# gcorso/disco-diffdock

Hardware: AMD Instinct MI355X
Metric: complexes/sec, 20-step 40-sample inference (higher is better)
Workload: dtype f32

## Files before the change

disco_diffdock_amd/csrc/conv_launch.hip:

```cpp
#include "k_conv_common.h"
#include "k_node.h"
#include "model.h"

namespace ddk {

__global__ void conv_setup_kernel(int32_t* tile_info, int g0, int g1, int g2, int g3, int g4) {
  if (threadIdx.x == 0 && blockIdx.x == 0) {
    const int go[5] = {g0, g1, g2, g3, g4};
    int ts = 0;
    tile_info[0] = 0;
    for (int g = 0; g < 4; ++g) {
      ts += (go[g + 1] - go[g] + 31) / 32;
      tile_info[g + 1] = ts;
    }
    for (int g = 0; g < 5; ++g) tile_info[5 + g] = go[g];
    tile_info[10] = 0;
  }
}

__global__ void conv_one_group_kernel(int32_t* gt, int n_groups, int k, int E) {
  const int g = threadIdx.x;
  if (g < n_groups) { gt[g] = 0; gt[n_groups + g] = g == k ? E : 0; }
}

// ... 164 lines not shown
}

static ConvXArgs conv_args(const ConvLayerDev& L, const ConvLaunch& a, bool f16, bool trace) {
  ConvXArgs X = {};
  ConvKArgs& k = X.k;
  k.x = a.x; k.src = a.src; k.dst = a.dst; k.edge_attr = a.edge_attr; k.sh = a.sh; k.sum = a.sum;
  k.counter = a.counter;
  k.b1p = L.b1p[0]; k.n_tiles = L.n_tiles;
  k.n_cols = L.n_cols;
  for (int c = 0; c <= L.n_cols; ++c) k.col_start[c] = L.col_start[c];
  k.sum_g2 = a.sum_g2; k.g2_node_off = a.g2_node_off;
  k.n_groups = a.n_groups; k.n_active = a.n_active; k.n_slots = a.n_slots; k.slots = a.slots; k.wmap = a.wmap;
  if (a.gbeg) { k.gbeg = a.gbeg; k.gend = a.gend; }
  else { k.gbeg = a.tile_info + 5; k.gend = a.tile_info + 6; }
  k.pre = a.pre; k.part = a.part; k.det_rng = a.det_rng; k.det_nr = a.det_nr;
  if (f16) {
    k.w1x = L.w1x; k.w1sx = L.w1sx; k.w2x = L.w2x;
    for (int g = 0; g < CONV_MAX_GROUPS; ++g) { k.w1s[g] = L.w1s[g]; k.w1u[g] = 1.0f / L.w1s[g]; k.w2s[g] = L.w2s[g]; k.w2u[g] = 1.0f / L.w2s[g]; }
  } else {
    k.w1p = L.w1p[0]; k.w2r = L.w2r[0];
    for (int g = 0; g < CONV_MAX_GROUPS; ++g) { k.w1s[g] = 1.0f; k.w1u[g] = 1.0f; k.w2s[g] = 1.0f; k.w2u[g] = 1.0f; }
  }
  X.trace = trace ? a.trace : nullptr; X.trace_coarse = a.trace_coarse;
  return X;
}

hipError_t conv_prepare_device() {
  for (int family = CONV_F32; family <= CONV_X2; ++family) {
    const ConvTable t = conv_table(family);
    for (int i = 0; i < t.n; ++i) {
// ... 30 lines not shown
```

disco_diffdock_amd/csrc/ddk_internal.h:

```cpp
#pragma once
#include <hip/hip_runtime.h>
#include <stdint.h>

#include <map>
#include <string>
#include <vector>

#include "../../include/ddk.h"
#include "../../include/ddk_debug.h"

namespace ddk {

constexpr int NS = 24;
constexpr int NV = 6;
constexpr int XW = 2 * NS + 6 * NV;
constexpr int NE = 3 * NS;
constexpr int OFF_P = NS;
constexpr int OFF_Q = NS + 3 * NV;
constexpr int OFF_C = NS + 6 * NV;

constexpr int F_A = 0;
constexpr int F_C = NS;
constexpr int F_T1O = 2 * NS;
constexpr int F_T1E = F_T1O + 6 * NV;
// ... 189 lines not shown
  const int32_t* src;
  const int32_t* dst;
  const float* edge_attr;
  const float* sh;
  float* sum;
  const int32_t* tile_info;
  int32_t* counter;
  float* part = nullptr;
  int64_t edge_bound = 0;
  const int32_t* det_rng = nullptr;
  int det_nr = 0;
  const float* pre = nullptr;
  int gather;
  float* sum_g2 = nullptr;
  int g2_node_off = 0;
  int mode = 0;
  int n_groups = 4, n_active = 4, n_slots = 1;
  uint32_t slots = 0;
  uint64_t wmap = 0x876543210ull;
  const int32_t* gbeg = nullptr;
  const int32_t* gend = nullptr;
  uint32_t* trace = nullptr;
  int trace_coarse = 0;
};
hipError_t launch_conv_fused(const ConvLayerDev& L, const ConvLaunch& a, int n_cu, hipStream_t s);
hipError_t launch_split3_probe(const float* x, int64_t n, int group, float* hi, float* mid, float* lo, float* scale, hipStream_t s);
int build_conv_layer(ddk_ctx* ctx, int mode, int l, ConvLayerDev& L);
int build_head_layer(ddk_ctx* ctx, int mode, ConvLayerDev& L);
hipError_t conv_prepare_device();
hipError_t graph_prepare_device(int* max_rec);
// ... 141 lines not shown
```

disco_diffdock_amd/csrc/k_conv.hip:

```cpp
#include <stdlib.h>

#include "k_conv_common.h"

namespace ddk {

__device__ __forceinline__ void load_frags(float4 (&a)[9], f32x16& B, const float* w, const float* b) {
#pragma unroll
  for (int s4 = 0; s4 < 9; ++s4) a[s4] = ld4(w + s4 * 256);
#pragma unroll
  for (int j = 0; j < 4; ++j) {
    const float4 v = ld4(b + 4 * j);
    B[4 * j + 0] = v.x; B[4 * j + 1] = v.y; B[4 * j + 2] = v.z; B[4 * j + 3] = v.w;
  }
}

__device__ __forceinline__ f32x16 burst(const float4 (&a)[9], const float (&h)[36], const f32x16& C) {
  f32x16 D = MFMA(a[0].x, h[0], C);
  D = MFMA(a[0].y, h[1], D);
  D = MFMA(a[0].z, h[2], D);
  D = MFMA(a[0].w, h[3], D);
#pragma unroll
  for (int s4 = 1; s4 < 9; ++s4) {
    D = MFMA(a[s4].x, h[4 * s4 + 0], D);
    D = MFMA(a[s4].y, h[4 * s4 + 1], D);
// ... 14 lines not shown
}

template <bool GATHER, int MODE, bool SPLIT, bool DET>
__global__ __launch_bounds__(64 * ConvTraits<MODE>::WAVES) void conv_fused_kernel(ConvKArgs A) {
  static_assert(!SPLIT || (GATHER && MODE == 0), "the GEMM1 split exists for the score model's gather path");
  static_assert(!DET || MODE == 0, "the deterministic scatter exists for the score model");
  constexpr int WAVES = ConvTraits<MODE>::WAVES, FS = ConvTraits<MODE>::FS, BLOCK_EDGES = 32 * WAVES;
  extern __shared__ __attribute__((aligned(16))) float lds[];
  const int tid = threadIdx.x, lane = tid & 63, wave = tid >> 6;
  float* F = lds + wave * (32 * FS);
  float* ring = lds + WAVES * (32 * FS);
  int* blk_slot = reinterpret_cast<int*>(ring + 2 * W2_TILE_FLOATS);
  const int el = lane & 31;
  const int hh = lane >> 5;
  const bool g2_shared = A.sum_g2 != nullptr;
  int gb_v = 0, ge_v = 0;
  if (lane < A.n_active) {
    gb_v = A.gbeg[lane];
    ge_v = A.gend[lane];
  }
  const int nb_v = (ge_v - gb_v + BLOCK_EDGES - 1) / BLOCK_EDGES;
  int pend_v = nb_v;
#pragma unroll
  for (int d = 1; d < 16; d *= 2) {
    const int t = __shfl_up(pend_v, d, 64);
    if (lane >= d) pend_v += t;
  }
  const int pbeg_v = pend_v - nb_v;
  int bs4 = __builtin_amdgcn_readlane(pend_v, 15);
  if constexpr (DET) {
// ... 32 lines not shown
    }
    int g = __popcll(__ballot(lane < 16 && blk >= pend_v));
    int gbeg = __builtin_amdgcn_readlane(gb_v, g), gend = __builtin_amdgcn_readlane(ge_v, g);
    int bstart = __builtin_amdgcn_readlane(pbeg_v, g);
    if constexpr (DET) {
      if (A.det_nr > 0) {
        const DetRange R_ = det_find(A.det_rng, A.det_nr, blk);
        g = R_.g; gbeg = R_.beg; gend = R_.end; bstart = R_.bstart;
      }
    }
    const int e0 = gbeg + BLOCK_EDGES * (blk - bstart) + 32 * wave;
    const int nvalid = min(32, gend - e0);
    const bool valid = el < nvalid;
    const int e = nvalid > 0 ? e0 + min(el, nvalid - 1) : gend - 1;
    const int sn = A.src[e], dn = A.dst[e];

    const int gw = (int)((A.wmap >> (4 * g)) & 15);
    const float* wrec = A.w2r + (size_t)gw * n_tiles * W2_TILE_FLOATS;
    {
      const float* wr0 = wrec + (size_t)t_begin * W2_TILE_FLOATS;
      const float* wr1 = wrec + (size_t)min(t_begin + 1, t_end - 1) * W2_TILE_FLOATS;
      const float4 r0 = ld4(wr0 + 4 * tid), r1 = ld4(wr1 + 4 * tid);
      *reinterpret_cast<float4*>(ring + 4 * tid) = r0;
      *reinterpret_cast<float4*>(ring + W2_TILE_FLOATS + 4 * tid) = r1;
      if (second) {
        const int q = 4 * (tid + 64 * WAVES);
        const float4 r2 = ld4(wr0 + q), r3 = ld4(wr1 + q);
        *reinterpret_cast<float4*>(ring + q) = r2;
        *reinterpret_cast<float4*>(ring + W2_TILE_FLOATS + q) = r3;
      }
    }

    const SegCtl seg = make_segctl(sn, el, nvalid, valid);

    float h[36];
    if constexpr (SPLIT) {
      float bin[12];
      {
        const float* pe = A.edge_attr + (size_t)e * NS + 12 * hh;
#pragma unroll
        for (int j = 0; j < 3; ++j) {
          const float4 a = ld4(pe + 4 * j);
          bin[4 * j + 0] = a.x; bin[4 * j + 1] = a.y; bin[4 * j + 2] = a.z; bin[4 * j + 3] = a.w;
        }
      }
      const float* ps = A.pre + ((size_t)sn * 4 + (gw & 1)) * NE + 36 * hh;
      const float* pd = A.pre + ((size_t)dn * 4 + 2 + (gw >> 1)) * NE + 36 * hh;
      const float* w1 = A.w1p + (size_t)gw * (3 * 9 * 64 * 4);
#pragma unroll
      for (int T = 0; T < 3; ++T) {
        f32x16 acc;
#pragma unroll
        for (int j = 0; j < 4; ++j) {
          if (T < 2 || j == 0) {
// ... 13 lines not shown
          acc = MFMA(a.w, bin[4 * s4 + 3], acc);
        }
        if (T < 2) {
#pragma unroll
          for (int r = 0; r < 16; ++r) h[16 * T + r] = fmaxf(acc[r], 0.0f);
        } else {
#pragma unroll
          for (int r = 0; r < 4; ++r) h[32 + r] = fmaxf(acc[r], 0.0f);
        }
      }
    } else {
    float bin[36];
    {
      const float *pe, *pxs, *pxd;
      if (GATHER) {
        pe = A.edge_attr + (size_t)e * NS + 12 * hh;
        pxs = A.x + (size_t)sn * XW + 12 * hh;
        pxd = A.x + (size_t)dn * XW + 12 * hh;
      } else {
        pe = A.edge_attr + (size_t)e * NE + 12 * hh;
        pxs = pe + NS;
        pxd = pe + 2 * NS;
      }
#pragma unroll
      for (int j = 0; j < 3; ++j) {
        const float4 a = ld4(pe + 4 * j), b = ld4(pxs + 4 * j), c = ld4(pxd + 4 * j);
        bin[4 * j + 0] = a.x; bin[4 * j + 1] = a.y; bin[4 * j + 2] = a.z; bin[4 * j + 3] = a.w;
        bin[12 + 4 * j + 0] = b.x; bin[12 + 4 * j + 1] = b.y; bin[12 + 4 * j + 2] = b.z; bin[12 + 4 * j + 3] = b.w;
        bin[24 + 4 * j + 0] = c.x; bin[24 + 4 * j + 1] = c.y; bin[24 + 4 * j + 2] = c.z; bin[24 + 4 * j + 3] = c.w;
      }
    }
// ... 17 lines not shown
          acc = MFMA(a.y, bin[4 * s4 + 1], acc);
          acc = MFMA(a.z, bin[4 * s4 + 2], acc);
          acc = MFMA(a.w, bin[4 * s4 + 3], acc);
        }
        if (T < 2) {
#pragma unroll
          for (int r = 0; r < 16; ++r) h[16 * T + r] = fmaxf(acc[r], 0.0f);
        } else {
#pragma unroll
          for (int r = 0; r < 4; ++r) h[32 + r] = fmaxf(acc[r], 0.0f);
        }
      }
    }
    }

    const float4 shv = ld4(A.sh + (size_t)e * 4);
    const float s0 = shv.x, vx = shv.y, vy = shv.z, vz = shv.w;
    {
      const float* xr = A.x + (size_t)dn * XW;
      const int o_main_src = hh ? OFF_C : 0, o_main_dst = hh ? F_C : F_A;
      const int o_vec_src = hh ? OFF_Q : OFF_P;
      const int o_vs = hh ? F_T1E : F_T1O, o_vc = hh ? F_T1O : F_T1E, r0 = hh ? NV : 0;
#pragma unroll
      for (int j = 0; j < NS / 4; ++j) *reinterpret_cast<float4*>(Fr + o_main_dst + 4 * j) = ld4(xr + o_main_src + 4 * j);
      float pv[3 * NV];
#pragma unroll
      for (int j = 0; j < 3 * NV / 2; ++j) {
        const float2 t = ld2(xr + o_vec_src + 2 * j);
        pv[2 * j] = t.x; pv[2 * j + 1] = t.y;
      }
#pragma unroll
// ... 135 lines not shown
```

disco_diffdock_amd/csrc/k_conv_common.h:

```cpp
#pragma once
#include "ddk_internal.h"

namespace ddk {

typedef float f32x16 __attribute__((ext_vector_type(16)));

struct ConvKArgs {
  const float* x;
  const int32_t* src;
  const int32_t* dst;
  const float* edge_attr;
  const float* sh;
  const float* pre;
  float* sum;
  int32_t* counter;
  const float* w1p;
  const float* b1p;
  const float* w2r;
  const uint8_t* w1x;
  const uint8_t* w1sx;
  const uint8_t* w2x;
  float w1s[CONV_MAX_GROUPS], w1u[CONV_MAX_GROUPS], w2s[CONV_MAX_GROUPS], w2u[CONV_MAX_GROUPS];
  int n_tiles;
  int n_cols;
  int col_start[17];
  float* part;
  float* sum_g2;
  int g2_node_off;
  int n_groups, n_active, n_slots;
  uint32_t slots;
  uint64_t wmap;
  const int32_t* gbeg;
  const int32_t* gend;
  const int32_t* det_rng = nullptr;
  int det_nr = 0;
};
struct DetRange { int beg, end, g, bstart; };
__device__ __forceinline__ DetRange det_find(const int32_t* rng, int nr, int blk) {
  int lo = 0, hi = nr;
  while (hi - lo > 1) {
    const int mid = (lo + hi) >> 1;
    if (rng[mid] <= blk) lo = mid; else hi = mid;
  }
  DetRange r;
  r.bstart = rng[lo]; r.beg = rng[nr + 1 + lo]; r.end = rng[2 * nr + 1 + lo]; r.g = rng[3 * nr + 1 + lo];
  return r;
}

struct ConvXArgs {
  ConvKArgs k;
// ... 125 lines not shown
```

disco_diffdock_amd/csrc/k_conv_x.hip:

```cpp
#include <stdlib.h>

#include "k_conv_common.h"

#ifdef X3_TWO_LIMBS
#define conv_x3_kernel conv_x2_kernel
#define conv_x3_table conv_x2_table
#include "k_conv_x_epi2_gen.inc"
#define X3_TILE_BYTES W2X2_TILE_BYTES
#define X3_BIAS_OFF W2X2_BIAS_OFF
#define X3_DESC_OFF W2X2_DESC_OFF
#define X3_W1_TILE_BYTES W1X2_TILE_BYTES
#define X3_LDS_BYTES CONV_X2_LDS_BYTES
#define X3_W1L_BYTES W1L_BYTES
#define X3_TWO true
#define X3_SUM(r) D0[r]
#define X3_TAIL3(a_lh, a_hm) (void)(a_lh); D0 = MFMA16(a_hm, HT.mh, D0); D0 = MFMA16(a_hm, HT.hm, D0);
#define X3_STEP(MF, ah, am, al, bh, bm, bl)   \
  (void)(al);                                 \
  D0 = MF(ah, bm, D0);                        \
  D0 = MF(am, bh, D0);                        \
  D0 = MF(ah, bh, D0);
#define X3_FRAG(f, off) f.h = *reinterpret_cast<const f16x8*>(ringl + (off)); f.m = *reinterpret_cast<const f16x8*>(ringl + W2X_LIMB_BYTES + (off));
#define X3_TAIL_LO(SO) th
#define X3_TRIO(mask) { __builtin_amdgcn_sched_group_barrier(0x008, 1, 0); __builtin_amdgcn_sched_group_barrier(mask, 1, 0); __builtin_amdgcn_sched_group_barrier(0x100, 1, 0); }
// ... 224 lines not shown
      if (slot == 2) ++trace_n;
    }
  };
  const ConvKArgs& A = AX.k;
  constexpr int WAVES = CONV_WAVES, FS = FX_STRIDE, BLOCK_EDGES = 32 * WAVES;
  extern __shared__ __attribute__((aligned(16))) float lds[];
  const int tid = threadIdx.x, lane = tid & 63, wave = tid >> 6;
  float* F = lds + wave * (32 * FS);
  char* ring = reinterpret_cast<char*>(lds + WAVES * (32 * FS));
  char* w1l = ring + W2X_STAGES * X3_TILE_BYTES;
  int* blk_slot = reinterpret_cast<int*>(w1l + X3_W1L_BYTES);
  (void)w1l;
  const int el = lane & 31;
  const int hh = lane >> 5;
  const bool g2_shared = A.sum_g2 != nullptr;
  int gb_v = 0, ge_v = 0;
  if (lane < A.n_active) {
    gb_v = A.gbeg[lane];
    ge_v = A.gend[lane];
  }
  const int nb_v = (ge_v - gb_v + BLOCK_EDGES - 1) / BLOCK_EDGES;
  int pend_v = nb_v;
#pragma unroll
  for (int d = 1; d < 16; d *= 2) {
    const int t = __shfl_up(pend_v, d, 64);
    if (lane >= d) pend_v += t;
  }
  const int pbeg_v = pend_v - nb_v;
  int bs4 = __builtin_amdgcn_readlane(pend_v, 15);
  if constexpr (DET) {
// ... 47 lines not shown
    }
    int g = __popcll(__ballot(lane < 16 && blk >= pend_v));
    int gbeg = __builtin_amdgcn_readlane(gb_v, g), gend = __builtin_amdgcn_readlane(ge_v, g);
    int bstart = __builtin_amdgcn_readlane(pbeg_v, g);
    if constexpr (DET) {
      if (A.det_nr > 0) {
        const DetRange R_ = det_find(A.det_rng, A.det_nr, blk);
        g = R_.g; gbeg = R_.beg; gend = R_.end; bstart = R_.bstart;
      }
    }
    const int e0 = gbeg + BLOCK_EDGES * (blk - bstart) + 32 * wave;
    const int nvalid = min(32, gend - e0);
    const bool valid = el < nvalid;
    const int e = nvalid > 0 ? e0 + min(el, nvalid - 1) : gend - 1;
    const int sn = A.src[e], dn = A.dst[e];

    const int gw = (int)((A.wmap >> (4 * g)) & 15);
    const char* wrec = reinterpret_cast<const char*>(A.w2x) + (size_t)gw * n_tiles * X3_TILE_BYTES;
    {
      const char* wr0 = wrec + (size_t)t_begin * X3_TILE_BYTES;
      const char* wr1 = wrec + (size_t)min(t_begin + 1, t_end - 1) * X3_TILE_BYTES;
      const char* wr2 = wrec + (size_t)min(t_begin + 2, t_end - 1) * X3_TILE_BYTES;
      const float4 r0 = *reinterpret_cast<const float4*>(wr0 + fo0);
      const float4 r2 = *reinterpret_cast<const float4*>(wr1 + fo0);
      const float4 r4 = *reinterpret_cast<const float4*>(wr2 + fo0);
      if (has1_s) { if (has1) {
        const float4 r1 = *reinterpret_cast<const float4*>(wr0 + fo1);
        const float4 r3 = *reinterpret_cast<const float4*>(wr1 + fo1);
        const float4 r5 = *reinterpret_cast<const float4*>(wr2 + fo1);
        *reinterpret_cast<float4*>(ring + fo1) = r1;
// ... 21 lines not shown
        gw_lds = gw_s;
        lds_barrier();
      }
    }
#endif

    const SegF seg = make_segf(make_segctl(sn, el, nvalid, valid));
    stamp(5);

    constexpr bool SENDK = SPLIT && X3_TWO;
    float4 shv;
    float4 mainv[NS / 4];
    float2 pv2[3 * NV / 2];
    const float* xr = A.x + (size_t)dn * XW;
    if constexpr (!SENDK) {
      shv = ld4(A.sh + (size_t)e * 4);
#pragma unroll
      for (int j = 0; j < NS / 4; ++j) mainv[j] = ld4(xr + (hh ? OFF_C : 0) + 4 * j);
#pragma unroll
      for (int j = 0; j < 3 * NV / 2; ++j) pv2[j] = ld2(xr + (hh ? OFF_Q : OFF_P) + 2 * j);
    }

    Limbs H;
    TailB HT;
    float osc, bsc2;
    {
      float h[36];
      const char* w1 = reinterpret_cast<const char*>(A.w1x) + (size_t)gw * 3 * X3_W1_TILE_BYTES;
      (void)w1;
      if constexpr (SPLIT) {
#ifdef X3_TWO_LIMBS
        float4 psv[9];
        {
          const float* ps = A.pre + ((size_t)sn * 4 + (gw & 1)) * NE + 36 * hh;
#pragma unroll
          for (int j = 0; j < 9; ++j) psv[j] = ld4(ps + 4 * j);
        }
        float bin[24];
        {
          const float* pe = A.edge_attr + (size_t)e * NS + 12 * hh;
#pragma unroll
          for (int j = 0; j < 3; ++j) {
            const float4 a = ld4(pe + 4 * j);
            bin[4 * j + 0] = a.x; bin[4 * j + 1] = a.y; bin[4 * j + 2] = a.z; bin[4 * j + 3] = a.w;
          }
#pragma unroll
          for (int j = 0; j < 3; ++j) mainv[j] = ld4(xr + 12 * hh + 4 * j);
        }
        shv = ld4(A.sh + (size_t)e * 4);
#pragma unroll
        for (int j = 0; j < 3; ++j) mainv[3 + j] = ld4(xr + OFF_C + 12 * hh + 4 * j);
#pragma unroll
        for (int j = 0; j < 3 * NV / 2; ++j) pv2[j] = ld2(xr + (hh ? OFF_Q : OFF_P) + 2 * j);
#pragma unroll
        for (int j = 0; j < 3; ++j) { bin[12 + 4 * j + 0] = mainv[j].x; bin[12 + 4 * j + 1] = mainv[j].y; bin[12 + 4 * j + 2] = mainv[j].z; bin[12 + 4 * j + 3] = mainv[j].w; }
        float m1 = 0.0f;
#pragma unroll
        for (int j = 0; j < 24; ++j) m1 = fmaxf(m1, fabsf(bin[j]));
        m1 = fmaxf(m1, __shfl_xor(m1, 32));
        float inv1;
        const float s1 = range_scale(m1, inv1);
        f16x8 bh[3], bm[3];
#pragma unroll
        for (int k = 0; k < 3; ++k)
// ... 21 lines not shown
          const int nr = T < 2 ? 16 : 4;
#pragma unroll
          for (int r = 0; r < 16; ++r)
            if (r < nr) h[16 * T + r] = fmaxf(D0[r], 0.0f) * usc;
        }
#else
        float4 psv[9], pdv[9];
        {
          const float* ps = A.pre + ((size_t)sn * 4 + (gw & 1)) * NE + 36 * hh;
          const float* pd = A.pre + ((size_t)dn * 4 + 2 + (gw >> 1)) * NE + 36 * hh;
#pragma unroll
          for (int j = 0; j < 9; ++j) { psv[j] = ld4(ps + 4 * j); pdv[j] = ld4(pd + 4 * j); }
        }
        float bin[12];
        {
          const float* pe = A.edge_attr + (size_t)e * NS + 12 * hh;
#pragma unroll
          for (int j = 0; j < 3; ++j) {
            const float4 a = ld4(pe + 4 * j);
            bin[4 * j + 0] = a.x; bin[4 * j + 1] = a.y; bin[4 * j + 2] = a.z; bin[4 * j + 3] = a.w;
          }
        }
        float m1 = 0.0f;
#pragma unroll
        for (int j = 0; j < 12; ++j) m1 = fmaxf(m1, fabsf(bin[j]));
        m1 = fmaxf(m1, __shfl_xor(m1, 32));
        float inv1;
        const float s1 = range_scale(m1, inv1);
        f16x8 b0h, b0m, b0l;
        f16x4 b1h, b1m, b1l;
#pragma unroll
// ... 25 lines not shown
            D0 = MFMA16(a_hm, b1_mh, D0);
            D1 = MFMA16(a_lh, b1_hl, D1);
            D0 = MFMA16(a_hm, b1_hm, D0);
          }
          const int nr = T < 2 ? 16 : 4;
#pragma unroll
          for (int r = 0; r < 16; ++r)
            if (r < nr) h[16 * T + r] = fmaxf(X3_SUM(r), 0.0f) * usc;
        }
#endif
      } else {
        float bin[36];
        {
          const float *pe, *pxs, *pxd;
          if (GATHER) {
            pe = A.edge_attr + (size_t)e * NS + 12 * hh;
            pxs = A.x + (size_t)sn * XW + 12 * hh;
            pxd = A.x + (size_t)dn * XW + 12 * hh;
          } else {
            pe = A.edge_attr + (size_t)e * NE + 12 * hh;
            pxs = pe + NS;
            pxd = pe + 2 * NS;
          }
#pragma unroll
          for (int j = 0; j < 3; ++j) {
            const float4 a = ld4(pe + 4 * j), b = ld4(pxs + 4 * j), c = ld4(pxd + 4 * j);
            bin[4 * j + 0] = a.x; bin[4 * j + 1] = a.y; bin[4 * j + 2] = a.z; bin[4 * j + 3] = a.w;
            bin[12 + 4 * j + 0] = b.x; bin[12 + 4 * j + 1] = b.y; bin[12 + 4 * j + 2] = b.z; bin[12 + 4 * j + 3] = b.w;
            bin[24 + 4 * j + 0] = c.x; bin[24 + 4 * j + 1] = c.y; bin[24 + 4 * j + 2] = c.z; bin[24 + 4 * j + 3] = c.w;
          }
        }
// ... 333 lines not shown
```

disco_diffdock_amd/csrc/k_graph.hip:

```cpp
#include <stdlib.h>
#include "model.h"
#include "k_node.h"

namespace ddk {


__device__ __forceinline__ bool cross_within(const float* lp, const float* rp, float c) {
#pragma clang fp contract(off)
  const float dx = rp[0] / c - lp[0] / c, dy = rp[1] / c - lp[1] / c, dz = rp[2] / c - lp[2] / c;
  return dx * dx + dy * dy + dz * dz < 1.0f;
}

__device__ __forceinline__ bool cross_within4(const float4 a, float rx, float ry, float rz) {
#pragma clang fp contract(off)
  const float dx = rx - a.x, dy = ry - a.y, dz = rz - a.z;
  return dx * dx + dy * dy + dz * dz < 1.0f;
}

__device__ __forceinline__ float dist2(const float* a, const float* b) {
#pragma clang fp contract(off)
  const float dx = a[0] - b[0], dy = a[1] - b[1], dz = a[2] - b[2];
  return dx * dx + dy * dy + dz * dz;
}

// ... 169 lines not shown
#pragma unroll
    for (int k = 0; k < 5; ++k) tot[k] += __shfl(inc[k], 63, 64);
  }
  ex[5] = b * G.E_rr - (ex[2] + ex[3] + ex[4]);
}

__device__ void write_group_tables(const GraphArgs& G, const int* tot) {
  const int ll = tot[0], lr = tot[1], ra = tot[2], rb = tot[3], rc = tot[4];
  int go[5];
  go[0] = 0; go[1] = ll; go[2] = ll + lr; go[3] = go[2] + G.B * G.E_rr; go[4] = go[3] + lr;
  const int seg[4] = {go[2], go[2] + ra, go[2] + ra + rb, go[2] + ra + rb + rc};
  const int n_shared = G.shared_rr ? G.E_rr : 0;
  int bs = 0;
  G.info[I_FB] = 0;
  for (int g = 0; g < 5; ++g) {
    bs += (g == 3 && G.cross_mirror) ? 0 : ((g < 4 ? go[g + 1] - go[g] : n_shared) + 255) / 256;
    G.info[I_FB + 1 + g] = bs;
  }
  for (int g = 0; g < 5; ++g) G.info[I_GO + g] = go[g];
  for (int k = 0; k < 8; ++k) G.info[I_CNT + k] = 0;
  for (int l = 0; l < 4; ++l) G.info[I_SEG + l] = seg[l];
  G.info[I_E] = go[4];
  G.info[I_OVF] = ((int64_t)go[4] + n_shared > G.edge_cap) ? 1 : 0;
  G.info[I_SHARED] = G.shared_rr ? go[4] : -1;
  G.info[I_HEAD] = 0; G.info[I_HEAD + 1] = G.B * G.n_lig; G.info[I_HEAD + 2] = G.B * G.n_lig; G.info[I_HEAD + 3] = G.B * G.n_lig;
  G.info[I_HEAD + 4] = 0; G.info[I_HEAD + 5] = 0;
  G.info[I_EXEC] = go[4];
  G.info[I_EXEC + 1] = go[2];
  G.info[I_EXEC + 7] = lr;
  for (int k = 0; k < N_TAB; ++k) {
    int32_t* tb = G.info + I_TAB + 8 * k;
// ... 571 lines not shown
```

disco_diffdock_amd/csrc/model.h:

```cpp
#pragma once
#include <stdio.h>
#include <stdlib.h>
#include <thread>

#include "ddk_internal.h"

namespace ddk {

constexpr int SIG = 32;
constexpr int DE = 32;
constexpr int MAX_LIG = 256;
constexpr int MAX_REC = 8192;
constexpr int LIG_CAP = 33;
constexpr int BOND_CAP = 32;
constexpr int LIG_DIMS[16] = {119, 4, 12, 12, 8, 10, 6, 6, 2, 8, 2, 2, 2, 2, 2, 2};
constexpr int REC_DIM = 38;

enum InfoSlot : int {
  I_GO = 5,
  I_CNT = 10,
  I_FB = 18,
  I_E = 24,
  I_OVF = 25,
  I_MISMATCH = 31,
// ... 109 lines not shown
  const int32_t* bond_src;
  const int32_t* bond_dst;
  const int32_t* rr_src;
  const int32_t* rr_dst;
  const int32_t* rr_outdeg;
  int B, n_lig, n_rec, M, E_rr;
  float lig_r2;
  float cross_cutoff;
  const int32_t* rr_start;
  int32_t* counts;
  int32_t* offs;
  int32_t* info;
  uint8_t* levels;
  int prune = 0;
  int shared_rr = 0;
  int32_t* e_src;
  int32_t* e_dst;
  int32_t* e_aux;
  int32_t* deg;
  int rec_node_base = -1;
  int64_t patch_off = -1;
  int64_t edge_cap = 0;
  int cross_mirror = 0;
};

int det_ranges_count(int kind, int B);
hipError_t launch_det_ranges(const GraphArgs& G, int kind, int len_uniform, int32_t* out, hipStream_t s);

struct PatchArgs {
  const float* rec_latent;
// ... 230 lines not shown
  int32_t* patch_cnt = nullptr;
  bool latent_dirty = true;
  int patch_B = 0;
  float cfg_weight = 0.0f, cfg_start = 1.0f, cfg_end = 0.0f;
  float *zero_lat = nullptr, *scores2 = nullptr;
  float* part = nullptr;
  int32_t* det_rng = nullptr;
  float* sum_rr0 = nullptr;
  int32_t *h_src = nullptr, *h_dst = nullptr, *h_deg = nullptr;
  float *h_attr = nullptr, *h_sh = nullptr, *h_sum = nullptr;
  float* pre = nullptr;
  float* x_last = nullptr;
  int last_B = 0;
  bool sum_clean = false;
  bool keep_rec = false, last_full = false;
  ddk::ConfComplex* conf = nullptr;
  ddk_ctx* owner = nullptr;
  struct Chunk { void* p; size_t cap; };
  std::vector<Chunk> allocs;
  char* chunk = nullptr;
  size_t chunk_cap = 0, chunk_off = 0, reserve_hint = 0;
  bool oom = false;
  int stage_idx = -1;
  size_t stage_off = 0;
  struct CopyRec { void* dst; size_t off, bytes; };
  std::vector<CopyRec> pending;
  hipEvent_t ready = nullptr;
  bool ready_pending = false;
  hipStream_t last_stream = nullptr;
  std::vector<hipStream_t> streams;
// ... 72 lines not shown
```

disco_diffdock_amd/csrc/model.hip:

```cpp
#include <math.h>
#include <string.h>

#include <algorithm>
#include <thread>

#include "k_philox.h"
#include "model.h"

namespace ddk {

std::vector<float> cols(const HostTensor* t, int c0, int c1) {
  const int rows = (int)t->shape[0], nc = (int)t->shape[1];
  std::vector<float> o((size_t)rows * (c1 - c0));
  for (int r = 0; r < rows; ++r)
    for (int c = c0; c < c1; ++c) o[(size_t)r * (c1 - c0) + (c - c0)] = t->data[(size_t)r * nc + c];
  return o;
}

static bool smearing(ddk_ctx* ctx, const char* name, float stop, EdgeMlpDev& m, std::vector<float>* host_off, float* host_coeff) {
  std::vector<float> off(DE);
  auto it = ctx->weights.find(std::string(name) + "_distance_expansion.offset");
  if (it != ctx->weights.end() && it->second.data.size() == (size_t)DE) off = it->second.data;
  else for (int k = 0; k < DE; ++k) off[k] = stop * (float)k / (float)(DE - 1);
  const double d = (double)(off[1] - off[0]);
// ... 390 lines not shown
  if (!cx->ready_pending) return hipSuccess;
  if (hipEventQuery(cx->ready) == hipSuccess) { cx->ready_pending = false; return hipSuccess; }
  return hipStreamWaitEvent(s, cx->ready, 0);
}

GraphArgs graph_args(const ddk_ctx* ctx, const ddk_complex* cx, int B, const float* lig_pos, float cross_cutoff) {
  GraphArgs G;
  G.lig_pos = lig_pos; G.rec_pos = cx->rec_pos; G.bond_src = cx->bond_src; G.bond_dst = cx->bond_dst;
  G.rr_src = cx->rr_src; G.rr_dst = cx->rr_dst; G.rr_outdeg = cx->rr_outdeg; G.rr_start = cx->rr_start;
  G.B = B; G.n_lig = cx->n_lig; G.n_rec = cx->n_rec; G.M = cx->M; G.E_rr = cx->E_rr;
  G.lig_r2 = ctx->cfg.lig_max_radius * ctx->cfg.lig_max_radius; G.cross_cutoff = cross_cutoff; G.counts = cx->counts; G.offs = cx->offs; G.info = cx->info; G.levels = cx->levels;
  return G;
}

static hipError_t build_graph(ddk_ctx* ctx, ddk_complex* cx, int B, const float* lig_pos, float cross_cutoff, bool prune, bool shared_rr,
                              hipStream_t s, int64_t patch_off = -1, int cross_mirror = 0) {
  GraphArgs G = graph_args(ctx, cx, B, lig_pos, cross_cutoff);
  G.cross_mirror = cross_mirror; G.prune = prune ? 1 : 0; G.shared_rr = shared_rr ? 1 : 0; G.patch_off = patch_off;
  G.e_src = cx->e_src; G.e_dst = cx->e_dst; G.e_aux = cx->e_aux; G.deg = cx->deg;
  return launch_graph(G, cx->edge_cap, s);
}

static int score_forward_impl(ddk_ctx* ctx, ddk_complex* cx, int B, const float* lig_pos, const StepParams& sp,
                              float* tr_out, float* rot_out, float* tor_out, hipStream_t s, HeadArgs* defer_post = nullptr) {
  const ddk_config& c = ctx->cfg;
  Model* M = (Model*)ctx->model;
  const int n_lig = cx->n_lig, n_rec = cx->n_rec;
  const int64_t N = (int64_t)B * (n_lig + n_rec);
  const bool patched = c.latent_dim > 0 && ctx->layer0_dedup && !c.deterministic && cx->patch_off >= 0 && cx->pre != nullptr &&
                       ctx->conv[0].wn != nullptr && c.num_conv_layers > 1;
  const bool dedup = ((c.latent_dim == 0 && ctx->layer0_dedup) || patched) && B > 1 && cx->E_rr > 0;
  if (c.latent_dim > 0 && (!cx->lig_latent || !cx->rec_latent))
    return fail(ctx, DDK_ERR_STATE, "latent-conditioned model: call ddk_set_latents before the forward");
  if (dedup && patched && (cx->latent_dirty || cx->patch_B != B)) {
    PatchArgs P;
    P.rec_latent = cx->rec_latent; P.rr_start = cx->rr_start; P.rr_outdeg = cx->rr_outdeg; P.rr_dst = cx->rr_dst;
    P.B = B; P.n_lig = n_lig; P.n_rec = n_rec; P.E_rr = cx->E_rr; P.latent_dim = c.latent_dim; P.patch_off = cx->patch_off;
    P.rr_mask = cx->rr_mask; P.patch_cnt = cx->patch_cnt; P.info = cx->info; P.e_src = cx->e_src; P.e_dst = cx->e_dst; P.e_aux = cx->e_aux;
    CK(launch_disco_patch(P, s), "layer-0 patch group");
    cx->latent_dirty = false; cx->patch_B = B;
  }
  const bool prune = ctx->prune && !cx->keep_rec && cx->E_rr > 0;
  const int mirror = graph_cross_mirror_fits(n_lig, n_rec);
  CK(build_graph(ctx, cx, B, lig_pos, sp.cross_cutoff, prune, dedup, s, (dedup && patched) ? cx->patch_off : -1, mirror), "graph build");
  EdgeFeatArgs F;
  F.cross_mirror = mirror;
  F.lig_pos = lig_pos; F.rec_pos = cx->rec_pos; F.bond_attr = cx->bond_attr; F.rr_pre1 = cx->rr_pre1; F.rr_sh = cx->rr_sh;
  F.e_src = cx->e_src; F.e_dst = cx->e_dst; F.e_aux = cx->e_aux; F.info = cx->info; F.e_emb = cx->e_emb; F.e_sh = cx->e_sh;
  F.lig = M->dev.lig_edge; F.rec = M->dev.rec_edge; F.cross = M->dev.cross_edge; F.sp = sp;
  F.n_lig_total = B * n_lig; F.n_rec = n_rec; F.n_shared = dedup ? cx->E_rr : 0;
  F.g2_live_only = (dedup && prune && c.num_conv_layers == 5) ? 1 : 0;
  F.patch_off = (dedup && patched) ? cx->patch_off : -1;
  F.latent_dim = c.latent_dim; F.lig_latent = cx->lig_latent; F.rec_latent = cx->rec_latent; F.unconditional = cx->unconditional;
  const int64_t cap_b = (int64_t)B * ((int64_t)cx->M + (int64_t)n_lig * LIG_CAP + 2LL * n_lig * n_rec + cx->E_rr) + cx->E_rr;
  const int64_t feat_cap = (cap_b < cx->edge_cap ? cap_b : cx->edge_cap) + (F.patch_off >= 0 ? (int64_t)B * cx->E_rr + 256 : 0);
  float* xin = cx->xa;
  float* xout = cx->xb;
  NodeEmbedArgs NE_;
  NE_.lig_static = cx->lig_node_static; NE_.rec_static = cx->rec_node_static; NE_.sp = sp; NE_.B = B; NE_.n_lig = n_lig; NE_.n_rec = n_rec;
  NE_.x = xin; NE_.lig_latent = cx->lig_latent; NE_.rec_latent = cx->rec_latent; NE_.lig_w_lat = M->dev.lig_w_lat; NE_.rec_w_lat = M->dev.rec_w_lat;
  NE_.lig_unc = M->dev.lig_node_unc; NE_.rec_unc = M->dev.rec_node_unc; NE_.unconditional = cx->unconditional; NE_.latent_dim = c.latent_dim;
  const bool split = ctx->conv[0].wn != nullptr && cx->pre != nullptr;
  const bool recv_only = split && ctx->conv[0].sender_in_gemm1;
  const int role_mask = recv_only ? 0x3 : 0xF;
  if (split) {
    NodePreArgs PA = {};
// ... 7 lines not shown
  if (!cx->sum_clean) {
    CK(hipMemsetAsync(cx->sum, 0, (size_t)cx->max_batch * (n_lig + n_rec) * XW * sizeof(float) * (c.deterministic ? 2 : 1), s), "memset sum");
    CK(hipMemsetAsync(cx->sum_rr0, 0, (size_t)n_rec * XW * sizeof(float), s), "memset sum_rr0");
  }
  cx->sum_clean = false;
  bool rr0_dirty = false;
  const int NL = c.num_conv_layers;
  int32_t* prof_slot = nullptr;
  if (ctx->prof && ctx->prof_slots + 1 <= ctx->prof_cap) prof_slot = ctx->prof_edges + (size_t)PROF_INTS * ctx->prof_slots;
  for (int l = 0; l < NL; ++l) {
    const ConvLayerDev& L = ctx->conv[l];
    ConvLaunch a;
    a.x = xin; a.src = cx->e_src; a.dst = cx->e_dst; a.edge_attr = cx->e_emb; a.sh = cx->e_sh; a.sum = cx->sum;
    a.tile_info = cx->info; a.counter = cx->info + I_CNT + (l % 8); a.gather = 1;
    a.pre = split ? cx->pre : nullptr;
    const bool lig_only = (l == NL - 1 && !cx->keep_rec);
    const bool shared0 = dedup && l == 0;
    int tab = TAB_ALL;
    if (shared0) tab = TAB_SHARED;
    else if (prune && l == NL - 2) tab = TAB_A;
    else if (prune && l == NL - 3) tab = TAB_B;
    else if (prune && l == NL - 4) tab = TAB_C;
    a.gbeg = cx->info + I_TAB + 8 * tab; a.gend = a.gbeg + 4;
    a.n_groups = 4; a.n_active = lig_only ? 2 : 4; a.n_slots = 1; a.slots = 0;
    if (shared0 && patched) {
      a.gbeg = cx->info + I_TABX; a.gend = a.gbeg + 5; a.n_groups = 5; a.n_active = 5; a.wmap = 0x23210ull;
    }
    if (c.deterministic) {
      a.n_slots = 2; a.slots = (0u) | (1u << 2) | (0u << 4) | (1u << 6);
      a.part = cx->part; a.edge_bound = cap_b;
// ... 839 lines not shown
  hipError_t e = launch_debug_axis_angle(aa, n, R_out, (hipStream_t)stream);
  return e == hipSuccess ? DDK_OK : hip_fail(ctx, e, "debug axis angle");
}

int ddk_debug_read_edges(ddk_ctx* ctx, ddk_complex* cx, int64_t first, int64_t n, int32_t* src, int32_t* dst, float* emb, float* sh, int32_t* deg,
                         int64_t n_nodes) {
  if (!ctx || !cx) return DDK_ERR_INVALID;
  const int64_t e_alloc = cx->edge_cap + (cx->patch_off >= 0 ? (int64_t)cx->max_batch * cx->E_rr : 0);
  if (first < 0 || n < 0 || first + n > e_alloc || n_nodes < 0 || n_nodes > (int64_t)cx->max_batch * (cx->n_lig + cx->n_rec))
    return fail(ctx, DDK_ERR_INVALID, "ddk_debug_read_edges: range outside the complex' edge / node arrays");
  hipError_t e = hipDeviceSynchronize();
  if (e == hipSuccess && src && n) e = hipMemcpy(src, cx->e_src + first, n * 4, hipMemcpyDeviceToHost);
  if (e == hipSuccess && dst && n) e = hipMemcpy(dst, cx->e_dst + first, n * 4, hipMemcpyDeviceToHost);
  if (e == hipSuccess && emb && n) e = hipMemcpy(emb, cx->e_emb + first * NS, n * NS * 4, hipMemcpyDeviceToHost);
  if (e == hipSuccess && sh && n) e = hipMemcpy(sh, cx->e_sh + first * 4, n * 16, hipMemcpyDeviceToHost);
  if (e == hipSuccess && deg && n_nodes) e = hipMemcpy(deg, cx->deg, n_nodes * 4, hipMemcpyDeviceToHost);
  return e == hipSuccess ? DDK_OK : hip_fail(ctx, e, "ddk_debug_read_edges");
}

int ddk_debug_cross_mirror(ddk_ctx* ctx, ddk_complex* cx) {
  if (!ctx || !cx) return DDK_ERR_INVALID;
  return graph_cross_mirror_fits(cx->n_lig, cx->n_rec) ? 1 : 0;
}

}
```

Before: 51.95.

## Share receptor-receptor edge features across batch via indexed table lookup

When there is no latent conditioning and the batch has more than one sample, rec-rec (group 2) edge embeddings and spherical harmonics are computed once into a shared table. The conv kernels then index that table through a per-edge aux id, and the per-sample group-2 feature blocks are no longer built. This removes repeated edge featurization over identical receptor edges, at the cost of an extra indirect load per edge and scattered reads into the table. The debug read path expands the table back into per-edge values.

```diff
diff --git a/disco_diffdock_amd/csrc/conv_launch.hip b/disco_diffdock_amd/csrc/conv_launch.hip
--- a/disco_diffdock_amd/csrc/conv_launch.hip
+++ b/disco_diffdock_amd/csrc/conv_launch.hip
@@ -202,6 +202,7 @@
   if (a.gbeg) { k.gbeg = a.gbeg; k.gend = a.gend; }
   else { k.gbeg = a.tile_info + 5; k.gend = a.tile_info + 6; }
   k.pre = a.pre; k.part = a.part; k.det_rng = a.det_rng; k.det_nr = a.det_nr;
+  if (a.gather && a.mode == 0 && a.aux != nullptr && a.attr_base != nullptr) { k.aux = a.aux; k.attr_base = a.attr_base; }
   if (f16) {
     k.w1x = L.w1x; k.w1sx = L.w1sx; k.w2x = L.w2x;
     for (int g = 0; g < CONV_MAX_GROUPS; ++g) { k.w1s[g] = L.w1s[g]; k.w1u[g] = 1.0f / L.w1s[g]; k.w2s[g] = L.w2s[g]; k.w2u[g] = 1.0f / L.w2s[g]; }
diff --git a/disco_diffdock_amd/csrc/ddk_internal.h b/disco_diffdock_amd/csrc/ddk_internal.h
--- a/disco_diffdock_amd/csrc/ddk_internal.h
+++ b/disco_diffdock_amd/csrc/ddk_internal.h
@@ -227,6 +227,8 @@
   int gather;
   float* sum_g2 = nullptr;
   int g2_node_off = 0;
+  const int32_t* aux = nullptr;
+  const int32_t* attr_base = nullptr;
   int mode = 0;
   int n_groups = 4, n_active = 4, n_slots = 1;
   uint32_t slots = 0;
diff --git a/disco_diffdock_amd/csrc/k_conv.hip b/disco_diffdock_amd/csrc/k_conv.hip
--- a/disco_diffdock_amd/csrc/k_conv.hip
+++ b/disco_diffdock_amd/csrc/k_conv.hip
@@ -52,6 +52,8 @@
   const int el = lane & 31;
   const int hh = lane >> 5;
   const bool g2_shared = A.sum_g2 != nullptr;
+  int attr_base = -1;
+  if constexpr (GATHER && MODE == 0 && !DET) { if (A.aux != nullptr) attr_base = *A.attr_base; }
   int gb_v = 0, ge_v = 0;
   if (lane < A.n_active) {
     gb_v = A.gbeg[lane];
@@ -114,6 +116,16 @@
     const bool valid = el < nvalid;
     const int e = nvalid > 0 ? e0 + min(el, nvalid - 1) : gend - 1;
     const int sn = A.src[e], dn = A.dst[e];
+    int ea = e;
+    if constexpr (GATHER && MODE == 0) {
+      const bool tab = attr_base >= 0 && g == 2 && !g2_shared;
+      if constexpr (DET) {
+        if (A.aux != nullptr && g == 2 && !g2_shared) ea = *A.attr_base + A.aux[e];
+      } else {
+        const int auxv = (tab ? A.aux : A.src)[e];
+        ea = tab ? attr_base + auxv : e;
+      }
+    }
 
     const int gw = (int)((A.wmap >> (4 * g)) & 15);
     const float* wrec = A.w2r + (size_t)gw * n_tiles * W2_TILE_FLOATS;
@@ -137,7 +149,7 @@
     if constexpr (SPLIT) {
       float bin[12];
       {
-        const float* pe = A.edge_attr + (size_t)e * NS + 12 * hh;
+        const float* pe = A.edge_attr + (size_t)ea * NS + 12 * hh;
 #pragma unroll
         for (int j = 0; j < 3; ++j) {
           const float4 a = ld4(pe + 4 * j);
@@ -181,7 +193,7 @@
     {
       const float *pe, *pxs, *pxd;
       if (GATHER) {
-        pe = A.edge_attr + (size_t)e * NS + 12 * hh;
+        pe = A.edge_attr + (size_t)ea * NS + 12 * hh;
         pxs = A.x + (size_t)sn * XW + 12 * hh;
         pxd = A.x + (size_t)dn * XW + 12 * hh;
       } else {
@@ -229,7 +241,7 @@
     }
     }
 
-    const float4 shv = ld4(A.sh + (size_t)e * 4);
+    const float4 shv = ld4(A.sh + (size_t)ea * 4);
     const float s0 = shv.x, vx = shv.y, vy = shv.z, vz = shv.w;
     {
       const float* xr = A.x + (size_t)dn * XW;
diff --git a/disco_diffdock_amd/csrc/k_conv_common.h b/disco_diffdock_amd/csrc/k_conv_common.h
--- a/disco_diffdock_amd/csrc/k_conv_common.h
+++ b/disco_diffdock_amd/csrc/k_conv_common.h
@@ -34,6 +34,8 @@
   const int32_t* gend;
   const int32_t* det_rng = nullptr;
   int det_nr = 0;
+  const int32_t* aux = nullptr;
+  const int32_t* attr_base = nullptr;
 };
 struct DetRange { int beg, end, g, bstart; };
 __device__ __forceinline__ DetRange det_find(const int32_t* rng, int nr, int blk) {
diff --git a/disco_diffdock_amd/csrc/k_conv_x.hip b/disco_diffdock_amd/csrc/k_conv_x.hip
--- a/disco_diffdock_amd/csrc/k_conv_x.hip
+++ b/disco_diffdock_amd/csrc/k_conv_x.hip
@@ -262,6 +262,8 @@
   const int el = lane & 31;
   const int hh = lane >> 5;
   const bool g2_shared = A.sum_g2 != nullptr;
+  int attr_base = -1;
+  if constexpr (GATHER && MODE == 0 && !DET) { if (A.aux != nullptr) attr_base = *A.attr_base; }
   int gb_v = 0, ge_v = 0;
   if (lane < A.n_active) {
     gb_v = A.gbeg[lane];
@@ -339,6 +341,16 @@
     const bool valid = el < nvalid;
     const int e = nvalid > 0 ? e0 + min(el, nvalid - 1) : gend - 1;
     const int sn = A.src[e], dn = A.dst[e];
+    int ea = e;
+    if constexpr (GATHER && MODE == 0) {
+      const bool tab = attr_base >= 0 && g == 2 && !g2_shared;
+      if constexpr (DET) {
+        if (A.aux != nullptr && g == 2 && !g2_shared) ea = *A.attr_base + A.aux[e];
+      } else {
+        const int auxv = (tab ? A.aux : A.src)[e];
+        ea = tab ? attr_base + auxv : e;
+      }
+    }
 
     const int gw = (int)((A.wmap >> (4 * g)) & 15);
     const char* wrec = reinterpret_cast<const char*>(A.w2x) + (size_t)gw * n_tiles * X3_TILE_BYTES;
@@ -390,7 +402,7 @@
     float2 pv2[3 * NV / 2];
     const float* xr = A.x + (size_t)dn * XW;
     if constexpr (!SENDK) {
-      shv = ld4(A.sh + (size_t)e * 4);
+      shv = ld4(A.sh + (size_t)ea * 4);
 #pragma unroll
       for (int j = 0; j < NS / 4; ++j) mainv[j] = ld4(xr + (hh ? OFF_C : 0) + 4 * j);
 #pragma unroll
@@ -414,7 +426,7 @@
         }
         float bin[24];
         {
-          const float* pe = A.edge_attr + (size_t)e * NS + 12 * hh;
+          const float* pe = A.edge_attr + (size_t)ea * NS + 12 * hh;
 #pragma unroll
           for (int j = 0; j < 3; ++j) {
             const float4 a = ld4(pe + 4 * j);
@@ -423,7 +435,7 @@
 #pragma unroll
           for (int j = 0; j < 3; ++j) mainv[j] = ld4(xr + 12 * hh + 4 * j);
         }
-        shv = ld4(A.sh + (size_t)e * 4);
+        shv = ld4(A.sh + (size_t)ea * 4);
 #pragma unroll
         for (int j = 0; j < 3; ++j) mainv[3 + j] = ld4(xr + OFF_C + 12 * hh + 4 * j);
 #pragma unroll
@@ -475,7 +487,7 @@
         }
         float bin[12];
         {
-          const float* pe = A.edge_attr + (size_t)e * NS + 12 * hh;
+          const float* pe = A.edge_attr + (size_t)ea * NS + 12 * hh;
 #pragma unroll
           for (int j = 0; j < 3; ++j) {
             const float4 a = ld4(pe + 4 * j);
@@ -531,7 +543,7 @@
         {
           const float *pe, *pxs, *pxd;
           if (GATHER) {
-            pe = A.edge_attr + (size_t)e * NS + 12 * hh;
+            pe = A.edge_attr + (size_t)ea * NS + 12 * hh;
             pxs = A.x + (size_t)sn * XW + 12 * hh;
             pxd = A.x + (size_t)dn * XW + 12 * hh;
           } else {
diff --git a/disco_diffdock_amd/csrc/k_graph.hip b/disco_diffdock_amd/csrc/k_graph.hip
--- a/disco_diffdock_amd/csrc/k_graph.hip
+++ b/disco_diffdock_amd/csrc/k_graph.hip
@@ -207,7 +207,7 @@
   int bs = 0;
   G.info[I_FB] = 0;
   for (int g = 0; g < 5; ++g) {
-    bs += (g == 3 && G.cross_mirror) ? 0 : ((g < 4 ? go[g + 1] - go[g] : n_shared) + 255) / 256;
+    bs += ((g == 3 && G.cross_mirror) || (g == 2 && G.g2_table && G.shared_rr)) ? 0 : ((g < 4 ? go[g + 1] - go[g] : n_shared) + 255) / 256;
     G.info[I_FB + 1 + g] = bs;
   }
   for (int g = 0; g < 5; ++g) G.info[I_GO + g] = go[g];
diff --git a/disco_diffdock_amd/csrc/model.h b/disco_diffdock_amd/csrc/model.h
--- a/disco_diffdock_amd/csrc/model.h
+++ b/disco_diffdock_amd/csrc/model.h
@@ -147,6 +147,7 @@
   uint8_t* levels;
   int prune = 0;
   int shared_rr = 0;
+  int g2_table = 0;
   int32_t* e_src;
   int32_t* e_dst;
   int32_t* e_aux;
@@ -407,6 +408,7 @@
   int last_B = 0;
   bool sum_clean = false;
   bool keep_rec = false, last_full = false;
+  bool rr_table = false;
   ddk::ConfComplex* conf = nullptr;
   ddk_ctx* owner = nullptr;
   struct Chunk { void* p; size_t cap; };
diff --git a/disco_diffdock_amd/csrc/model.hip b/disco_diffdock_amd/csrc/model.hip
--- a/disco_diffdock_amd/csrc/model.hip
+++ b/disco_diffdock_amd/csrc/model.hip
@@ -428,9 +428,9 @@
 }
 
 static hipError_t build_graph(ddk_ctx* ctx, ddk_complex* cx, int B, const float* lig_pos, float cross_cutoff, bool prune, bool shared_rr,
-                              hipStream_t s, int64_t patch_off = -1, int cross_mirror = 0) {
+                              hipStream_t s, int64_t patch_off = -1, int cross_mirror = 0, bool g2_table = false) {
   GraphArgs G = graph_args(ctx, cx, B, lig_pos, cross_cutoff);
-  G.cross_mirror = cross_mirror; G.prune = prune ? 1 : 0; G.shared_rr = shared_rr ? 1 : 0; G.patch_off = patch_off;
+  G.cross_mirror = cross_mirror; G.prune = prune ? 1 : 0; G.shared_rr = shared_rr ? 1 : 0; G.patch_off = patch_off; G.g2_table = (g2_table && shared_rr) ? 1 : 0;
   G.e_src = cx->e_src; G.e_dst = cx->e_dst; G.e_aux = cx->e_aux; G.deg = cx->deg;
   return launch_graph(G, cx->edge_cap, s);
 }
@@ -456,14 +456,16 @@
   }
   const bool prune = ctx->prune && !cx->keep_rec && cx->E_rr > 0;
   const int mirror = graph_cross_mirror_fits(n_lig, n_rec);
-  CK(build_graph(ctx, cx, B, lig_pos, sp.cross_cutoff, prune, dedup, s, (dedup && patched) ? cx->patch_off : -1, mirror), "graph build");
+  const bool rr_table = c.latent_dim == 0 && B > 1 && cx->E_rr > 0;
+  cx->rr_table = rr_table;
+  CK(build_graph(ctx, cx, B, lig_pos, sp.cross_cutoff, prune, dedup || rr_table, s, (dedup && patched) ? cx->patch_off : -1, mirror, rr_table), "graph build");
   EdgeFeatArgs F;
   F.cross_mirror = mirror;
   F.lig_pos = lig_pos; F.rec_pos = cx->rec_pos; F.bond_attr = cx->bond_attr; F.rr_pre1 = cx->rr_pre1; F.rr_sh = cx->rr_sh;
   F.e_src = cx->e_src; F.e_dst = cx->e_dst; F.e_aux = cx->e_aux; F.info = cx->info; F.e_emb = cx->e_emb; F.e_sh = cx->e_sh;
   F.lig = M->dev.lig_edge; F.rec = M->dev.rec_edge; F.cross = M->dev.cross_edge; F.sp = sp;
-  F.n_lig_total = B * n_lig; F.n_rec = n_rec; F.n_shared = dedup ? cx->E_rr : 0;
-  F.g2_live_only = (dedup && prune && c.num_conv_layers == 5) ? 1 : 0;
+  F.n_lig_total = B * n_lig; F.n_rec = n_rec; F.n_shared = (dedup || rr_table) ? cx->E_rr : 0;
+  F.g2_live_only = (!rr_table && dedup && prune && c.num_conv_layers == 5) ? 1 : 0;
   F.patch_off = (dedup && patched) ? cx->patch_off : -1;
   F.latent_dim = c.latent_dim; F.lig_latent = cx->lig_latent; F.rec_latent = cx->rec_latent; F.unconditional = cx->unconditional;
   const int64_t cap_b = (int64_t)B * ((int64_t)cx->M + (int64_t)n_lig * LIG_CAP + 2LL * n_lig * n_rec + cx->E_rr) + cx->E_rr;
@@ -501,6 +503,7 @@
     a.x = xin; a.src = cx->e_src; a.dst = cx->e_dst; a.edge_attr = cx->e_emb; a.sh = cx->e_sh; a.sum = cx->sum;
     a.tile_info = cx->info; a.counter = cx->info + I_CNT + (l % 8); a.gather = 1;
     a.pre = split ? cx->pre : nullptr;
+    if (rr_table) { a.aux = cx->e_aux; a.attr_base = cx->info + I_SHARED; }
     const bool lig_only = (l == NL - 1 && !cx->keep_rec);
     const bool shared0 = dedup && l == 0;
     int tab = TAB_ALL;
@@ -1370,6 +1373,24 @@
   if (e == hipSuccess && dst && n) e = hipMemcpy(dst, cx->e_dst + first, n * 4, hipMemcpyDeviceToHost);
   if (e == hipSuccess && emb && n) e = hipMemcpy(emb, cx->e_emb + first * NS, n * NS * 4, hipMemcpyDeviceToHost);
   if (e == hipSuccess && sh && n) e = hipMemcpy(sh, cx->e_sh + first * 4, n * 16, hipMemcpyDeviceToHost);
+  if (e == hipSuccess && cx->rr_table && (emb || sh) && n) {
+    int32_t info[INFO_INTS];
+    e = hipMemcpy(info, cx->info, sizeof(info), hipMemcpyDeviceToHost);
+    const int64_t lo = std::max<int64_t>(first, info[I_GO + 2]), hi = std::min<int64_t>(first + n, info[I_GO + 3]), base = info[I_SHARED];
+    if (e == hipSuccess && lo < hi && base >= 0 && base + cx->E_rr <= e_alloc) {
+      std::vector<int32_t> aux((size_t)(hi - lo));
+      std::vector<float> temb((size_t)cx->E_rr * NS), tsh((size_t)cx->E_rr * 4);
+      e = hipMemcpy(aux.data(), cx->e_aux + lo, aux.size() * 4, hipMemcpyDeviceToHost);
+      if (e == hipSuccess) e = hipMemcpy(temb.data(), cx->e_emb + base * NS, temb.size() * 4, hipMemcpyDeviceToHost);
+      if (e == hipSuccess) e = hipMemcpy(tsh.data(), cx->e_sh + base * 4, tsh.size() * 4, hipMemcpyDeviceToHost);
+      for (int64_t i = lo; e == hipSuccess && i < hi; ++i) {
+        const int32_t k = aux[(size_t)(i - lo)];
+        if (k < 0 || k >= cx->E_rr) return fail(ctx, DDK_ERR_STATE, "ddk_debug_read_edges: a rec-rec edge without a static id");
+        if (emb) memcpy(emb + (i - first) * NS, temb.data() + (size_t)k * NS, NS * 4);
+        if (sh) memcpy(sh + (i - first) * 4, tsh.data() + (size_t)k * 4, 16);
+      }
+    }
+  }
   if (e == hipSuccess && deg && n_nodes) e = hipMemcpy(deg, cx->deg, n_nodes * 4, hipMemcpyDeviceToHost);
   return e == hipSuccess ? DDK_OK : hip_fail(ctx, e, "ddk_debug_read_edges");
 }
```

After: 51.98 (median of 2 runs). About the same (+0.1%).
